# eora-ai/torchok

Measured on AMD Instinct MI355X. Metric: images/sec (node) ResNet-50 224px bs256/GPU; step p50 ms, higher is better.
Workload: dtype bf16

## Files before the change

### torchok_amd/csrc/conv_wgrad.hip

```cpp
#include "tok_common.h"
#include "conv_common.h"
#include <type_traits>
#include <stdlib.h>

namespace {

struct WgradArgs {
  const bf16* x;
  const bf16* dy;
  float* ws;
  int H, W, C, K, R, S, P, Q, stride, pad;
  int M, PQ, HW, Ktot;
  int tilesN, tilesK, splitM, mchunk;
  uint32_t x_bytes, dy_bytes;
  uint32_t pq_mul, pq_shift, q_mul, q_shift;
  float* cs;
  int cs_cols;
  int adv_q, adv_p;
  size_t cs_stride, ws_stride;
};

__device__ __forceinline__ uint32_t magic_div(uint32_t n, uint32_t mul, uint32_t shift) {
  return (uint32_t)(((uint64_t)__umulhi(n, mul) + n) >> shift);
}
// ... 663 lines not shown
  for (int st = 0; st < steps; ++st) {
    asm volatile("s_waitcnt vmcnt(%0) lgkmcnt(0)" ::"n"(LOADS) : "memory");
    __builtin_amdgcn_s_barrier();
    issue(nxt);
    const uint32_t Yb = lds_base + cur * STAGE + rbase;
    const uint32_t Xb = Yb + TILE;
    u32x2 ya[NT][2], xb[KTL][2];
#pragma unroll
    for (int i = 0; i < NT; ++i) {
      ya[i][0] = tr_read_asm(Yb + colb(i));
      ya[i][1] = tr_read_asm(Yb + 16 * 128 + colb(i));
    }
#pragma unroll
    for (int j = 0; j < KTL; ++j) {
      const int J = wv * KTL + j;
      const uint32_t ad = Xb + (uint32_t)((J >> 2) * TILE) + colb(J & 3);
      xb[j][0] = tr_read_asm(ad);
      xb[j][1] = tr_read_asm(ad + 16 * 128);
    }
    bf16x8 af[NT];
    asm volatile("s_waitcnt lgkmcnt(%0)" ::"n"(2 * (KTL - 5)) : "memory");
    __builtin_amdgcn_sched_barrier(0);
#pragma unroll
    for (int i = 0; i < NT; ++i) af[i] = __builtin_bit_cast(bf16x8, (u32x4){ya[i][0][0], ya[i][0][1], ya[i][1][0], ya[i][1][1]});
#pragma unroll
    for (int j = 0; j < 5; ++j) {
      const bf16x8 bfr = __builtin_bit_cast(bf16x8, (u32x4){xb[j][0][0], xb[j][0][1], xb[j][1][0], xb[j][1][1]});
#pragma unroll
      for (int i = 0; i < NT; ++i) acc[i][j] = __builtin_amdgcn_mfma_f32_16x16x32_bf16(af[i], bfr, acc[i][j], 0, 0, 0);
    }
    __builtin_amdgcn_sched_barrier(0);
    asm volatile("s_waitcnt lgkmcnt(0)" ::: "memory");
    __builtin_amdgcn_sched_barrier(0);
#pragma unroll
    for (int j = 5; j < KTL; ++j) {
      const bf16x8 bfr = __builtin_bit_cast(bf16x8, (u32x4){xb[j][0][0], xb[j][0][1], xb[j][1][0], xb[j][1][1]});
#pragma unroll
      for (int i = 0; i < NT; ++i) acc[i][j] = __builtin_amdgcn_mfma_f32_16x16x32_bf16(af[i], bfr, acc[i][j], 0, 0, 0);
    }
    cur = cur == NST - 1 ? 0 : cur + 1;
    nxt = nxt == NST - 1 ? 0 : nxt + 1;
  }
  asm volatile("s_waitcnt vmcnt(0)" ::: "memory");

  float* out = a.ws + (size_t)split * a.K * a.Ktot;
#pragma unroll
  for (int j = 0; j < KTL; ++j) {
    const int J = wv * KTL + j;
    const int cin = ct * TC + (J & 3) * 16 + li;
    const int kcol = (J >> 2) * a.C + cin;
#pragma unroll
    for (int i = 0; i < NT; ++i)
#pragma unroll
      for (int r = 0; r < 4; ++r) {
        const int n = tn * TN + i * 16 + g * 4 + r;
        if (n < a.K && cin < a.C) out[(size_t)n * a.Ktot + kcol] = acc[i][j][r];
      }
  }
}


template <int CT, int NST, int KTLP>
__global__ __launch_bounds__(256, 2) void conv_wgrad_winp_kernel(WgradArgs a) {
  constexpr int MS = 32, TN = 16 * CT, TC = 16 * CT, TAPS = 9;
  constexpr int WIN = MS + 2;
  constexpr int YT = MS * 128;
  constexpr int XT = 128 * 128;
  constexpr int STAGE = YT + XT;
  constexpr int LOADS = 1 + 4;
  constexpr int NT = CT, KTL = KTLP;
  constexpr int NTILES = TAPS * CT;
  constexpr int NCW = (NTILES + KTL - 1) / KTL;
  static_assert(NCW == 4 && KTL >= 7 && NST >= 3, "four compute waves");

  extern __shared__ __attribute__((aligned(16))) char smem[];

  const int tid = threadIdx.x;
  const int lane = tid & 63;
  const int wv = __builtin_amdgcn_readfirstlane(tid >> 6);

  const int tilesC = a.tilesK;
  const int ntile = a.tilesN * tilesC;
  const int id = tok_xcd_remap(blockIdx.x, ntile * a.splitM);
  const int split = id / ntile;
  const int t = id - split * ntile;
  const int tn = t / tilesC;
  const int ct = t - tn * tilesC;

  const int mstart = split * a.mchunk;
  const int mend = min(a.M, mstart + a.mchunk);
  const int steps = (mend - mstart + MS - 1) / MS;

  auto run = [&](auto WVC) {
  const int row = tid >> 3, cc = tid & 7;
  const int clog = cc ^ ((row & 3) << 1);
  const int yn = tn * TN + clog * 8;
  const bool yn_ok = yn < a.K && clog * 8 < TN;
  const int cx = ct * TC + clog * 8;
  const bool cx_ok = cx < a.C && clog * 8 < TC;
  uint32_t doff[LOADS];
  const uint32_t dinc_y = (uint32_t)(MS * a.K) * 2u;
  const uint32_t dinc_x = (uint32_t)(MS * a.C) * 2u;
  doff[0] = yn_ok ? (uint32_t)((mstart + row) * a.K + yn) * 2u : 0xC0000000u;
#pragma unroll
  for (int j = 0; j < 4; ++j) {
    const int R = row + 32 * j;
    const int win = R / WIN;
    const bool live = cx_ok && R < 3 * WIN;
    const int pix = mstart + (win - 1) * a.W - 1 + (R - win * WIN);
    doff[1 + j] = live ? (uint32_t)(pix * a.C + cx) * 2u : 0xC0000000u;
  }

  const __amdgpu_buffer_rsrc_t ysrd = __builtin_amdgcn_make_buffer_rsrc((void*)a.dy, 0, a.dy_bytes, 0x00020000);
  const __amdgpu_buffer_rsrc_t xsrd = __builtin_amdgcn_make_buffer_rsrc((void*)a.x, 0, a.x_bytes, 0x00020000);
  typedef __attribute__((address_space(3))) void lds_void;

  auto issue_piece = [&](int slot, int pc) {
    char* base = smem + slot * STAGE + wv * 1024;
    if (pc == 0) __builtin_amdgcn_raw_ptr_buffer_load_lds(ysrd, (lds_void*)base, 16, doff[0], 0, 0, 0);
    else __builtin_amdgcn_raw_ptr_buffer_load_lds(xsrd, (lds_void*)(base + YT + (pc - 1) * 4096), 16, doff[pc], 0, 0, 0);
    doff[pc] += pc == 0 ? dinc_y : dinc_x;
  };

  const int rrow = 4 * (lane >> 4) + ((lane & 15) >> 2);
  const uint32_t cq = (uint32_t)((lane & 3) * 8);
  typedef __attribute__((address_space(3))) char lds_char;
  const uint32_t lds_base = (uint32_t)(size_t)(lds_char*)smem;
  const uint32_t yrc = (uint32_t)(rrow * 128) | cq | (uint32_t)(((rrow & 3) << 1) << 4);

  int pp[2], qq[2], mm0 = mstart + rrow;
#pragma unroll
  for (int h = 0; h < 2; ++h) {
    const uint32_t mc = (uint32_t)min(mm0 + 16 * h, a.M - 1);
    const uint32_t b = magic_div(mc, a.pq_mul, a.pq_shift);
    const uint32_t rem = mc - b * (uint32_t)a.PQ;
    const uint32_t p0 = magic_div(rem, a.q_mul, a.q_shift);
    pp[h] = (int)p0; qq[h] = (int)(rem - p0 * (uint32_t)a.Q);
  }
  const int mend16 = mend - 16;

  constexpr int W0 = decltype(WVC)::value;
  constexpr int T0 = (W0 * KTL) / CT;
  auto tap_of = [](int j) constexpr { return (W0 * KTL + j) / CT - T0; };
  auto last_j = [&](int k) constexpr { int l = -1; for (int j = 0; j < KTL && W0 * KTL + j < NTILES; ++j) if (tap_of(j) == k) l = j; return l; };
  uint32_t xrc[3];
#pragma unroll
  for (int k = 0; k < 3; ++k) {
    const int tap = T0 + k < TAPS ? T0 + k : TAPS - 1;
    const int kr = tap / 3, ks = tap - kr * 3;
    const int R = kr * WIN + ks + rrow;
    xrc[k] = (uint32_t)(R * 128) | cq | (uint32_t)(((R & 3) << 1) << 4);
  }
  f32x4 acc[NT][KTL];
#pragma unroll
  for (int i = 0; i < NT; ++i)
#pragma unroll
    for (int j = 0; j < KTL; ++j) acc[i][j] = (f32x4){0.f, 0.f, 0.f, 0.f};

  auto bases_tap = [&](int slot, int k, uint32_t (&tb)[3][2]) {
    const uint32_t Xb = lds_base + slot * STAGE + YT;
    const uint32_t zero_line = Xb + 127 * 128;
    const int tap = T0 + k < TAPS ? T0 + k : TAPS - 1;
    const int kr = tap / 3, ks = tap - kr * 3;
#pragma unroll
    for (int h = 0; h < 2; ++h) {
      bool ok = h == 0 ? mm0 < mend : mm0 < mend16;
      if (kr == 0) ok = ok && pp[h] >= 1;
      if (kr == 2) ok = ok && pp[h] <= a.H - 2;
      if (ks == 0) ok = ok && qq[h] >= 1;
      if (ks == 2) ok = ok && qq[h] <= a.W - 2;
      tb[k][h] = ok ? xrc[k] + (Xb + (uint32_t)(h * 16 * 128)) : zero_line;
    }
  };
  auto advance = [&]() {
#pragma unroll
    for (int h = 0; h < 2; ++h) {
      int q = qq[h] + a.adv_q;
      const bool wq = q >= a.Q;
      q -= wq ? a.Q : 0;
      int p = pp[h] + a.adv_p + (wq ? 1 : 0);
      p -= p >= a.P ? a.P : 0;
      qq[h] = q; pp[h] = p;
    }
    mm0 += MS;
  };
  auto read_y = [&](int slot, int i, u32x2 (&ya)[NT][2]) {
    const uint32_t ad = (yrc + (lds_base + slot * STAGE)) ^ (uint32_t)(i * 32);
    asm volatile("ds_read_b64_tr_b16 %0, %1" : "=v"(ya[i][0]) : "v"(ad));
    asm volatile("ds_read_b64_tr_b16 %0, %1 offset:2048" : "=v"(ya[i][1]) : "v"(ad));
  };
  auto read_x = [&](const uint32_t (&tb)[3][2], int j, u32x2 (&xb)[KTL][2]) {
    if (W0 * KTL + j >= NTILES) return;
    const int J = W0 * KTL + j;
    const int k = J / CT - T0;
    const uint32_t tl = (uint32_t)((J % CT) * 32);
    xb[j][0] = tr_read_asm(tb[k][0] ^ tl);
    xb[j][1] = tr_read_asm(tb[k][1] ^ tl);
  };

  u32x2 yA[NT][2], yB[NT][2], xb[KTL][2];
  uint32_t tb[3][2];

#pragma unroll
  for (int s_ = 0; s_ < NST; ++s_)
#pragma unroll
    for (int pc = 0; pc < LOADS; ++pc) issue_piece(s_, pc);
  asm volatile("s_waitcnt vmcnt(%0)" ::"n"((NST - 1) * LOADS) : "memory");
  __builtin_amdgcn_s_barrier();
#pragma unroll
  for (int k = 0; k < 3; ++k) bases_tap(0, k, tb);
#pragma unroll
  for (int i = 0; i < NT; ++i) read_y(0, i, yA);
#pragma unroll
  for (int j = 0; j < KTL; ++j) read_x(tb, j, xb);
  advance();
#pragma unroll
  for (int k = 0; k < 3; ++k) bases_tap(1 % NST, k, tb);
  int rd = 1 % NST, wr = 0;

  auto body = [&](u32x2 (&ycur)[NT][2], u32x2 (&ynxt)[NT][2]) {
    asm volatile("s_waitcnt vmcnt(%0) lgkmcnt(0)" ::"n"((NST - 2) * LOADS) : "memory");
    __builtin_amdgcn_s_barrier();
    __builtin_amdgcn_sched_barrier(0);
    const int rd2 = rd == NST - 1 ? 0 : rd + 1;
    bf16x8 af[NT];
#pragma unroll
    for (int i = 0; i < NT; ++i) af[i] = __builtin_bit_cast(bf16x8, (u32x4){ycur[i][0][0], ycur[i][0][1], ycur[i][1][0], ycur[i][1][1]});
#pragma unroll
    for (int j = 0; j < KTL; ++j) {
      if (W0 * KTL + j < NTILES) {
        const bf16x8 bfr = __builtin_bit_cast(bf16x8, (u32x4){xb[j][0][0], xb[j][0][1], xb[j][1][0], xb[j][1][1]});
#pragma unroll
        for (int i = 0; i < NT; ++i) acc[i][j] = __builtin_amdgcn_mfma_f32_16x16x32_bf16(af[i], bfr, acc[i][j], 0, 0, 0);
      }
      if (j < LOADS) issue_piece(wr, j);
      if (j == 0) advance();
      if (j >= 1 && (j - 1) * 2 < NT) { read_y(rd, (j - 1) * 2, ynxt); if ((j - 1) * 2 + 1 < NT) read_y(rd, (j - 1) * 2 + 1, ynxt); }
      read_x(tb, j, xb);
#pragma unroll
      for (int k = 0; k < 3; ++k)
        if (last_j(k) == j) bases_tap(rd2, k, tb);
      __builtin_amdgcn_sched_barrier(0);
    }
    rd = rd2;
    wr = wr == NST - 1 ? 0 : wr + 1;
  };
  for (int st = 0; st < steps; st += 2) {
    body(yA, yB);
    if (st + 1 < steps) body(yB, yA);
  }
  asm volatile("s_waitcnt vmcnt(0) lgkmcnt(0)" ::: "memory");

  int lane2;
  asm volatile("v_mbcnt_lo_u32_b32 %0, -1, 0\n\tv_mbcnt_hi_u32_b32 %0, -1, %0" : "=v"(lane2));
  const int g = lane2 >> 4, li = lane2 & 15;
  float* out = a.ws + (size_t)split * a.K * a.Ktot;
#pragma unroll
  for (int j = 0; j < KTL; ++j) {
    const int J = W0 * KTL + j;
    if (J >= NTILES) continue;
    const int cin = ct * TC + (J % CT) * 16 + li;
    const int kcol = (J / CT) * a.C + cin;
#pragma unroll
    for (int i = 0; i < NT; ++i)
#pragma unroll
      for (int r = 0; r < 4; ++r) {
        const int n = tn * TN + i * 16 + g * 4 + r;
        if (n < a.K && cin < a.C) out[(size_t)n * a.Ktot + kcol] = acc[i][j][r];
      }
  }
  };
  if (wv == 0) run(std::integral_constant<int, 0>{});
  else if (wv == 1) run(std::integral_constant<int, 1>{});
  else if (wv == 2) run(std::integral_constant<int, 2>{});
  else run(std::integral_constant<int, 3>{});
}

__global__ void wgrad_reduce_kernel(const float* __restrict__ ws, float* __restrict__ dw, int splitM,
                                    int k_real, int R, int S, int c_real, int K, int S_pad,
                                    int C_pad, int accumulate) {
  const size_t total = (size_t)k_real * R * S * c_real;
  const size_t slab = (size_t)K * R * S_pad * C_pad;
  for (size_t i = (size_t)blockIdx.x * blockDim.x + threadIdx.x; i < total;
       i += (size_t)gridDim.x * blockDim.x) {
    const int c = (int)(i % c_real);
    size_t rest = i / c_real;
    const int s = (int)(rest % S);
    rest /= S;
    const int r = (int)(rest % R);
    const int k = (int)(rest / R);
    const size_t src = (((size_t)k * R + r) * S_pad + s) * C_pad + c;
    float t = 0.f;
    for (int sp = 0; sp < splitM; sp += 8) {
      float v[8];
#pragma unroll
      for (int u = 0; u < 8; ++u) v[u] = ws[(size_t)(sp + u < splitM ? sp + u : splitM - 1) * slab + src];
#pragma unroll
      for (int u = 0; u < 8; ++u) t += sp + u < splitM ? v[u] : 0.f;
    }
    dw[i] = accumulate ? dw[i] + t : t;
  }
}

template <int U>
__device__ __forceinline__ void reduce_slabs(const float* __restrict__ ws, size_t stride, size_t i, int row, int splitM, float4& t) {
  for (int sp = row; sp < splitM; sp += 16 * U) {
    float4 v[U];
#pragma unroll
    for (int u = 0; u < U; ++u) {
      const int su = sp + 16 * u;
      v[u] = reinterpret_cast<const float4*>(ws + (size_t)(su < splitM ? su : splitM - 1) * stride)[i];
    }
#pragma unroll
    for (int u = 0; u < U; ++u) {
      if (sp + 16 * u < splitM) { t.x += v[u].x; t.y += v[u].y; t.z += v[u].z; t.w += v[u].w; }
    }
  }
}

__global__ __launch_bounds__(256) void wgrad_reduce_flat_kernel(const float* __restrict__ ws, float* __restrict__ dw,
                                                                int splitM, size_t slab, int accumulate, size_t stride,
                                                                float* __restrict__ extra, int extra_n, int extra_pad,
                                                                int extra_acc) {
  __shared__ float4 red[16][16];
  const int col = threadIdx.x & 15, row = threadIdx.x >> 4;
  const size_t m4 = slab >> 2;
  const size_t n4 = m4 + (extra != nullptr ? (size_t)(extra_pad >> 2) : 0);
  for (size_t base = (size_t)blockIdx.x * 16; base < n4; base += (size_t)gridDim.x * 16) {
    const size_t i = base + col;
    float4 t = {0.f, 0.f, 0.f, 0.f};
    if (i < n4) {
      if (splitM > 64) reduce_slabs<8>(ws, stride, i, row, splitM, t);
      else if (splitM > 32) reduce_slabs<4>(ws, stride, i, row, splitM, t);
      else if (splitM > 16) reduce_slabs<2>(ws, stride, i, row, splitM, t);
      else if (row < splitM) {
        const float4 v = reinterpret_cast<const float4*>(ws + (size_t)row * stride)[i];
        t.x += v.x; t.y += v.y; t.z += v.z; t.w += v.w;
      }
    }
    red[row][col] = t;
    __syncthreads();
    for (int s_ = 8; s_ > 0; s_ >>= 1) {
      if (row < s_) {
        const float4 o = red[row + s_][col];
        float4 m = red[row][col];
        m.x += o.x; m.y += o.y; m.z += o.z; m.w += o.w;
        red[row][col] = m;
      }
      __syncthreads();
    }
    if (row == 0 && i < m4) {
      float4 r = red[0][col];
      if (accumulate) {
        const float4 o = reinterpret_cast<const float4*>(dw)[i];
        r.x += o.x; r.y += o.y; r.z += o.z; r.w += o.w;
      }
      reinterpret_cast<float4*>(dw)[i] = r;
    } else if (row == 0 && i < n4) {
      const float4 r = red[0][col];
      const float rv[4] = {r.x, r.y, r.z, r.w};
      const int e0 = (int)(i - m4) * 4;
#pragma unroll
      for (int e = 0; e < 4; ++e)
        if (e0 + e < extra_n) extra[e0 + e] = extra_acc ? extra[e0 + e] + rv[e] : rv[e];
    }
    __syncthreads();
  }
}

struct Plan {
  int TN, TK, tilesN, tilesK, splitM, mchunk, MS;
  bool ring;
  bool taps;
};

static int taps_target() {
  static const int v = [] { const char* e = getenv("TOK_WGRAD_TAPS_WGS"); return (int)(e ? atoi(e) : 256); }();
  return v;
}

static int ring_target() {
  static const int v = [] { const char* e = getenv("TOK_WGRAD_WGS"); return (int)(e ? atoi(e) : 0); }();
  return v;
}

Plan make_plan(const tok_conv_desc* d) {
  Plan p;
  const int Ktot = d->r * d->s_pad * d->c;
  const long long M = (long long)d->n * d->p * d->q;
  p.taps = false;
  const bool same3 = d->r == 3 && d->s == 3 && d->s_pad == 3 && d->stride == 1 && d->pad == 1 &&
                     (unsigned long long)d->n * d->h * d->w * d->c * 2 < 0x40000000ull &&
                     (unsigned long long)d->n * d->p * d->q * d->k * 2 < 0x40000000ull;
  const bool w64 = d->c % 64 == 0 && d->k % 64 == 0;
  const bool w48 = !w64 && d->c % 48 == 0 && d->k % 48 == 0 && same3;
  if (d->c != 4 && (w64 || w48) && d->r == 3 && d->s == 3 && d->s_pad == 3) {
    p.taps = true; p.ring = false;
    p.TN = w64 ? 64 : 48; p.TK = p.TN; p.MS = 32;
    p.tilesN = tok_cdiv(d->k, p.TN);
    p.tilesK = tok_cdiv(d->c, p.TN);
    const int tiles = p.tilesN * p.tilesK;
    long long split = (taps_target() + tiles - 1) / tiles;
    const long long max_split = (M + 8 * 32 - 1) / (8 * 32);
    if (split > max_split) split = max_split;
    if (split > 512) split = 512;
    if (split < 1) split = 1;
    long long chunk = (M + split - 1) / split;
    chunk = ((chunk + 31) / 32) * 32;
    p.mchunk = (int)chunk;
    p.splitM = (int)((M + chunk - 1) / chunk);
    return p;
  }
  p.ring = d->c != 4 && d->r == 1 && d->s == 1 && d->stride == 1 && d->pad == 0;
  if (p.ring) {
    p.MS = 32;
    if (d->k <= 64) { p.TN = 64; p.TK = Ktot >= 256 ? 256 : (Ktot >= 128 ? 128 : 64); }
    else if (Ktot <= 64) { p.TK = 64; p.TN = d->k >= 256 ? 256 : 128; }
    else { p.TN = 128; p.TK = 128; }
    static const int big = [] { const char* e = getenv("TOK_WGRAD_256"); return (int)(e ? atoi(e) : 1); }();
    if (big && d->r == 1 && d->s == 1 && d->stride == 1 && d->pad == 0 && d->k >= 256 && Ktot >= 256 && M >= (big >= 2 ? 8192 : 200000) &&
        (long long)tok_cdiv(d->k, 256) * tok_cdiv(Ktot, 256) * 65536 * 2 <= (long long)d->k * Ktot * 3) {
      p.TN = 256; p.TK = 256;
    }
    p.tilesN = tok_cdiv(d->k, p.TN);
    p.tilesK = tok_cdiv(Ktot, p.TK);
    const int tiles = p.tilesN * p.tilesK;
    const int stage = 32 * (p.TN + p.TK) * 2;
    const int per_cu = (160 * 1024) / (3 * stage);
    static const int long_target = [] { const char* e = getenv("TOK_WGRAD_WGS_LONG"); return (int)(e ? atoi(e) : 0); }();
    const int target = (long_target > 0 && M >= 100000) ? long_target
                       : ring_target() > 0 ? ring_target() : 256 * (per_cu > 2 ? 2 : per_cu);
    long long split = (target + tiles - 1) / tiles;
    const long long max_split = (M + 8 * 32 - 1) / (8 * 32);
    if (split > max_split) split = max_split;
    if (split > 512) split = 512;
    if (split < 1) split = 1;
    long long chunk = (M + split - 1) / split;
    chunk = ((chunk + 31) / 32) * 32;
    p.mchunk = (int)chunk;
    p.splitM = (int)((M + chunk - 1) / chunk);
    return p;
  }
  p.TN = d->k >= 128 ? 128 : 64;
  p.TK = Ktot >= 128 ? 128 : 64;
  p.tilesN = tok_cdiv(d->k, p.TN);
  p.tilesK = tok_cdiv(Ktot, p.TK);
  const int tiles = p.tilesN * p.tilesK;
  static const int tb_target = [] { const char* e = getenv("TOK_WGRAD_2BUF_WGS"); return (int)(e ? atoi(e) : 1024); }();
  long long split = (tb_target + tiles - 1) / tiles;
  p.MS = (M >= 100000 && p.TN == 128 && p.TK == 128) ? 64 : 32;
  const long long max_split = (M + 8 * p.MS - 1) / (8 * p.MS);
  if (split > max_split) split = max_split;
  const long long cap = (d->c == 4 && tiles <= 2) ? 512 : 256;
  if (split > cap) split = cap;
  if (split < 1) split = 1;
  long long chunk = (M + split - 1) / split;
  chunk = ((chunk + p.MS - 1) / p.MS) * p.MS;
  p.mchunk = (int)chunk;
  p.splitM = (int)((M + chunk - 1) / chunk);
  return p;
}

template <int TN, int TK>
void launch_ring(const WgradArgs& a, hipStream_t st) {
  constexpr int smem = 3 * 32 * (TN + TK) * 2;
  static const bool attr_set = [&] {
    (void)hipFuncSetAttribute(reinterpret_cast<const void*>(&conv_wgrad_ring_kernel<TN, TK>),
                              hipFuncAttributeMaxDynamicSharedMemorySize, smem);
    return true;
  }();
  (void)attr_set;
  hipLaunchKernelGGL((conv_wgrad_ring_kernel<TN, TK>), dim3(a.tilesN * a.tilesK * a.splitM), dim3(256), smem, st, a);
}

template <int TN, int TK, bool C4, int MS, bool PWK>
void launch_wgrad_pw(const WgradArgs& a, hipStream_t st) {
  constexpr int smem = 2 * MS * ((TN + 16) * 2 + (TK + 16) * 2);
  static const bool attr_set = [&] {
    (void)hipFuncSetAttribute(reinterpret_cast<const void*>(&conv_wgrad_kernel<TN, TK, C4, MS, PWK>),
                              hipFuncAttributeMaxDynamicSharedMemorySize, smem);
    return true;
  }();
  (void)attr_set;
  hipLaunchKernelGGL((conv_wgrad_kernel<TN, TK, C4, MS, PWK>), dim3(a.tilesN * a.tilesK * a.splitM), dim3(256),
                     smem, st, a);
}

template <int TN, int TK, bool C4, int MS>
void launch_wgrad_ms(const WgradArgs& a, hipStream_t st) {
  if constexpr (!C4) {
    if (a.R == 1 && a.S == 1 && a.stride == 1 && a.pad == 0) { launch_wgrad_pw<TN, TK, C4, MS, true>(a, st); return; }
  }
  launch_wgrad_pw<TN, TK, C4, MS, false>(a, st);
}

template <int TN, int TK, bool C4>
void launch_wgrad(const WgradArgs& a, hipStream_t st, int ms) {
  if (ms == 64) launch_wgrad_ms<TN, TK, C4, 64>(a, st);
  else launch_wgrad_ms<TN, TK, C4, 32>(a, st);
}

}

extern "C" size_t tok_conv_wgrad_ws_bytes(const tok_conv_desc* d) {
  if (d == nullptr) return 0;
  const Plan p = make_plan(d);
  return (size_t)p.splitM * d->k * d->r * d->s_pad * d->c * sizeof(float);
}

extern "C" int tok_conv_wgrad_bias_ok(const tok_conv_desc* d) {
  if (d == nullptr || d->c == 4) return 0;
  return make_plan(d).ring ? 1 : 0;
}

extern "C" size_t tok_conv_wgrad_bias_ws_bytes(const tok_conv_desc* d) {
  if (d == nullptr) return 0;
  const Plan p = make_plan(d);
  return tok_conv_wgrad_ws_bytes(d) + (size_t)p.splitM * d->k * sizeof(float);
}

namespace {
int wgrad_impl(const tok_conv_desc* d, const void* x, const void* dy, float* dw, int k_real, int c_real, void* ws, size_t ws_bytes,
               int accumulate, float* dbias, int bias_accumulate, void* stream);
}

extern "C" int tok_conv_wgrad(const tok_conv_desc* d, const void* x, const void* dy, float* dw,
                              int k_real, int c_real, void* ws, size_t ws_bytes, int accumulate,
                              void* stream) {
  return wgrad_impl(d, x, dy, dw, k_real, c_real, ws, ws_bytes, accumulate, nullptr, 0, stream);
}

extern "C" int tok_conv_wgrad_bias(const tok_conv_desc* d, const void* x, const void* dy, float* dw, int k_real, int c_real,
                                   void* ws, size_t ws_bytes, int accumulate, float* dbias, int bias_accumulate, void* stream) {
  TOK_CHECK_ARG(dbias != nullptr, "tok_conv_wgrad_bias: dbias must not be null");
  TOK_CHECK_ARG(tok_conv_wgrad_bias_ok(d), "tok_conv_wgrad_bias: layer not served (ask tok_conv_wgrad_bias_ok)");
  return wgrad_impl(d, x, dy, dw, k_real, c_real, ws, ws_bytes, accumulate, dbias, bias_accumulate, stream);
}

namespace {
int wgrad_impl(const tok_conv_desc* d, const void* x, const void* dy, float* dw, int k_real, int c_real, void* ws, size_t ws_bytes,
               int accumulate, float* dbias, int bias_accumulate, void* stream) {
  TOK_CHECK_ARG(d && x && dy && dw && ws, "tok_conv_wgrad: null pointer");
  if (tok_dbg_skip(16)) return TOK_OK;
  TOK_CHECK_ARG(d->k % 8 == 0 && (d->c % 8 == 0 || d->c == 4), "tok_conv_wgrad: bad channel padding");
  TOK_CHECK_ARG(k_real <= d->k && c_real <= d->c, "tok_conv_wgrad: real dims exceed padded dims");
  TOK_CHECK_ARG(d->c == 4 ? d->s_pad == 8 : d->s_pad == d->s, "tok_conv_wgrad: bad s_pad");
  const Plan p = make_plan(d);
  const size_t need = dbias ? tok_conv_wgrad_bias_ws_bytes(d) : tok_conv_wgrad_ws_bytes(d);
  if (ws_bytes < need) {
    tok_set_error("tok_conv_wgrad: workspace %zu < %zu bytes", ws_bytes, need);
    return TOK_ERR_WORKSPACE;
  }
  const bool flat = (k_real == d->k) && (c_real == d->c) && (d->s_pad == d->s) &&
                    (((size_t)d->k * d->r * d->s * d->c) % 4 == 0) && (((uintptr_t)dw & 15) == 0);
  const bool direct = flat && p.splitM == 1 && !accumulate;
  WgradArgs a;
  a.x = (const bf16*)x; a.dy = (const bf16*)dy; a.ws = direct ? dw : (float*)ws;
  a.H = d->h; a.W = d->w; a.C = d->c; a.K = d->k; a.R = d->r; a.S = d->s_pad; a.P = d->p; a.Q = d->q;
  a.stride = d->stride; a.pad = d->pad;
  a.M = d->n * d->p * d->q; a.PQ = d->p * d->q; a.HW = d->h * d->w;
  make_magic((uint32_t)a.PQ, a.pq_mul, a.pq_shift);
  make_magic((uint32_t)d->q, a.q_mul, a.q_shift);
  a.adv_q = 32 % d->q; a.adv_p = (32 / d->q) % d->p;
  a.Ktot = d->r * d->s_pad * d->c;
  a.tilesN = p.tilesN; a.tilesK = p.tilesK; a.splitM = p.splitM; a.mchunk = p.mchunk;
  const size_t slab_f = (size_t)d->k * d->r * d->s_pad * d->c;
  const int cs_pad = (k_real + 3) / 4 * 4;
  const bool cs_inline = dbias != nullptr && flat && !direct;
  a.ws_stride = cs_inline ? slab_f + cs_pad : slab_f;
  a.cs = dbias ? (cs_inline ? (float*)ws + slab_f : (float*)((char*)ws + tok_conv_wgrad_ws_bytes(d))) : nullptr;
  a.cs_stride = cs_inline ? a.ws_stride : (size_t)k_real;
  a.cs_cols = k_real;
  {
    const unsigned long long xb = (unsigned long long)d->n * d->h * d->w * d->c * 2;
    const unsigned long long yb = (unsigned long long)a.M * d->k * 2;
    TOK_CHECK_ARG(xb < 0xFFFFFFF0ull && yb < 0xFFFFFFF0ull, "tok_conv_wgrad: tensors of 4 GiB or more are not supported");
    a.x_bytes = (uint32_t)xb; a.dy_bytes = (uint32_t)yb;
  }
  hipStream_t st = tok_stream(stream);
  const bool c4 = d->c == 4;
  if (c4 && dbias == nullptr && stem_wgrad_serves(d)) {
    stem_wgrad_launch(d, x, dy, a.ws, p.splitM, st);
  } else
  if (p.taps) {
    constexpr int smem = 3 * 10 * 32 * 128;
    static const bool attr_set = [&] {
      (void)hipFuncSetAttribute(reinterpret_cast<const void*>(&conv_wgrad_taps_kernel<0>),
                                hipFuncAttributeMaxDynamicSharedMemorySize, smem);
      return true;
    }();
    (void)attr_set;
    const bool same = a.stride == 1 && a.pad == 1 && a.P == a.H && a.Q == a.W && a.x_bytes < 0x40000000u && a.dy_bytes < 0x40000000u;
    if (same) {
      constexpr int smem_p = 3 * (32 * 128 + 128 * 128);
      static const bool attr_p = [&] {
        (void)hipFuncSetAttribute(reinterpret_cast<const void*>(&conv_wgrad_winp_kernel<4, 3, 9>), hipFuncAttributeMaxDynamicSharedMemorySize, smem_p);
        (void)hipFuncSetAttribute(reinterpret_cast<const void*>(&conv_wgrad_winp_kernel<3, 3, 7>), hipFuncAttributeMaxDynamicSharedMemorySize, smem_p);
        return true;
      }();
      (void)attr_p;
      const dim3 gw(a.tilesN * a.tilesK * a.splitM);
      if (p.TN == 48) hipLaunchKernelGGL((conv_wgrad_winp_kernel<3, 3, 7>), gw, dim3(256), smem_p, st, a);
      else hipLaunchKernelGGL((conv_wgrad_winp_kernel<4, 3, 9>), gw, dim3(256), smem_p, st, a);
    } else {
      hipLaunchKernelGGL((conv_wgrad_taps_kernel<0>), dim3(a.tilesN * a.tilesK * a.splitM), dim3(256), smem, st, a);
    }
  } else if (p.ring) {
    if (p.TN == 256 && p.TK == 256) {
      constexpr int smem8 = 3 * 32 * (256 + 256) * 2;
      static const bool attr8 = [] {
        (void)hipFuncSetAttribute(reinterpret_cast<const void*>(&conv_wgrad_ring8_kernel<256, 256>),
                                  hipFuncAttributeMaxDynamicSharedMemorySize, smem8);
        return true;
      }();
      (void)attr8;
      hipLaunchKernelGGL((conv_wgrad_ring8_kernel<256, 256>), dim3(a.tilesN * a.tilesK * a.splitM), dim3(512), smem8, st, a);
    }
    else if (p.TN == 64 && p.TK == 64) launch_ring<64, 64>(a, st);
    else if (p.TN == 64 && p.TK == 128) launch_ring<64, 128>(a, st);
    else if (p.TN == 64 && p.TK == 256) launch_ring<64, 256>(a, st);
    else if (p.TN == 128 && p.TK == 64) launch_ring<128, 64>(a, st);
    else if (p.TN == 256 && p.TK == 64) launch_ring<256, 64>(a, st);
    else launch_ring<128, 128>(a, st);
  } else if (p.TN == 128 && p.TK == 128) {
    if (c4) launch_wgrad<128, 128, true>(a, st, p.MS); else launch_wgrad<128, 128, false>(a, st, p.MS);
  } else if (p.TN == 128) {
    if (c4) launch_wgrad<128, 64, true>(a, st, p.MS); else launch_wgrad<128, 64, false>(a, st, p.MS);
  } else if (p.TK == 128) {
    if (c4) launch_wgrad<64, 128, true>(a, st, p.MS); else launch_wgrad<64, 128, false>(a, st, p.MS);
  } else {
    if (c4) launch_wgrad<64, 64, true>(a, st, p.MS); else launch_wgrad<64, 64, false>(a, st, p.MS);
  }
  TOK_CHECK_LAUNCH("tok_conv_wgrad");
  if (dbias != nullptr && !cs_inline) {
    if (int e = tok_colsum_f32(a.cs, p.splitM, k_real, dbias, bias_accumulate, stream)) return e;
  }
  if (direct) return TOK_OK;
  if (flat) {
    if (tok_dbg_skip(2)) return TOK_OK;
    const size_t slab = (size_t)d->k * d->r * d->s * d->c;
    const size_t nb = (slab / 4 + 15) / 16;
    hipLaunchKernelGGL(wgrad_reduce_flat_kernel, dim3((int)(nb < 4096 ? nb : 4096)), dim3(256), 0, st,
                       (const float*)ws, dw, p.splitM, slab, accumulate, cs_inline ? a.ws_stride : slab,
                       cs_inline ? dbias : (float*)nullptr, k_real, cs_inline ? cs_pad : 0, bias_accumulate);
    TOK_CHECK_LAUNCH("tok_conv_wgrad(reduce)");
    return TOK_OK;
  }
  const size_t total = (size_t)k_real * d->r * d->s * c_real;
  const int blocks = (int)((total + 255) / 256 < 2048 ? (total + 255) / 256 : 2048);
  hipLaunchKernelGGL(wgrad_reduce_kernel, dim3(blocks), dim3(256), 0, st, (const float*)ws, dw,
                     p.splitM, k_real, d->r, d->s, c_real, d->k, d->s_pad, d->c, accumulate);
  TOK_CHECK_LAUNCH("tok_conv_wgrad(reduce)");
  return TOK_OK;
}
}
```

Baseline: 14600.

## Rewrite split-M wgrad reduction as per-thread register fold without shared memory

Replaces the shared-memory tree reduction of split-M workspace slabs with a kernel where each thread owns V contiguous outputs and folds all slabs itself into 16 register accumulators, followed by an in-register tree. Vector width (1/2/4) and unroll depth are chosen on the host from the output size and splitM, so small layers get more threads. This removes __syncthreads and LDS traffic and launches one thread per output vector instead of a grid-stride loop. In exchange, each thread serially reads every slab, which lowers parallelism when splitM is large and raises register pressure.

```diff
diff --git a/torchok_amd/csrc/conv_wgrad.hip b/torchok_amd/csrc/conv_wgrad.hip
--- a/torchok_amd/csrc/conv_wgrad.hip
+++ b/torchok_amd/csrc/conv_wgrad.hip
@@ -989,70 +989,84 @@
   }
 }
 
-template <int U>
-__device__ __forceinline__ void reduce_slabs(const float* __restrict__ ws, size_t stride, size_t i, int row, int splitM, float4& t) {
-  for (int sp = row; sp < splitM; sp += 16 * U) {
-    float4 v[U];
-#pragma unroll
-    for (int u = 0; u < U; ++u) {
-      const int su = sp + 16 * u;
-      v[u] = reinterpret_cast<const float4*>(ws + (size_t)(su < splitM ? su : splitM - 1) * stride)[i];
-    }
-#pragma unroll
-    for (int u = 0; u < U; ++u) {
-      if (sp + 16 * u < splitM) { t.x += v[u].x; t.y += v[u].y; t.z += v[u].z; t.w += v[u].w; }
-    }
-  }
-}
-
+template <int V> struct FoldVec;
+template <> struct FoldVec<1> { float f[1]; };
+template <> struct alignas(8) FoldVec<2> { float f[2]; };
+template <> struct alignas(16) FoldVec<4> { float f[4]; };
+
+template <int V, int B, bool TAIL>
+__device__ __forceinline__ void fold_round(const float* __restrict__ src, size_t stride, int sp, int splitM, float (&acc)[16][V]) {
+  FoldVec<V> v[B];
+#pragma unroll
+  for (int u = 0; u < B; ++u) {
+    const int s = TAIL && sp + u >= splitM ? splitM - 1 : sp + u;
+    v[u] = *reinterpret_cast<const FoldVec<V>*>(src + (size_t)s * stride);
+  }
+#pragma unroll
+  for (int u = 0; u < B; ++u) {
+    if (!TAIL || sp + u < splitM) {
+#pragma unroll
+      for (int j = 0; j < V; ++j) acc[u & 15][j] += v[u].f[j];
+    }
+  }
+}
+
+template <int V, int B>
 __global__ __launch_bounds__(256) void wgrad_reduce_flat_kernel(const float* __restrict__ ws, float* __restrict__ dw,
                                                                 int splitM, size_t slab, int accumulate, size_t stride,
                                                                 float* __restrict__ extra, int extra_n, int extra_pad,
                                                                 int extra_acc) {
-  __shared__ float4 red[16][16];
-  const int col = threadIdx.x & 15, row = threadIdx.x >> 4;
-  const size_t m4 = slab >> 2;
-  const size_t n4 = m4 + (extra != nullptr ? (size_t)(extra_pad >> 2) : 0);
-  for (size_t base = (size_t)blockIdx.x * 16; base < n4; base += (size_t)gridDim.x * 16) {
-    const size_t i = base + col;
-    float4 t = {0.f, 0.f, 0.f, 0.f};
-    if (i < n4) {
-      if (splitM > 64) reduce_slabs<8>(ws, stride, i, row, splitM, t);
-      else if (splitM > 32) reduce_slabs<4>(ws, stride, i, row, splitM, t);
-      else if (splitM > 16) reduce_slabs<2>(ws, stride, i, row, splitM, t);
-      else if (row < splitM) {
-        const float4 v = reinterpret_cast<const float4*>(ws + (size_t)row * stride)[i];
-        t.x += v.x; t.y += v.y; t.z += v.z; t.w += v.w;
-      }
-    }
-    red[row][col] = t;
-    __syncthreads();
-    for (int s_ = 8; s_ > 0; s_ >>= 1) {
-      if (row < s_) {
-        const float4 o = red[row + s_][col];
-        float4 m = red[row][col];
-        m.x += o.x; m.y += o.y; m.z += o.z; m.w += o.w;
-        red[row][col] = m;
-      }
-      __syncthreads();
-    }
-    if (row == 0 && i < m4) {
-      float4 r = red[0][col];
-      if (accumulate) {
-        const float4 o = reinterpret_cast<const float4*>(dw)[i];
-        r.x += o.x; r.y += o.y; r.z += o.z; r.w += o.w;
-      }
-      reinterpret_cast<float4*>(dw)[i] = r;
-    } else if (row == 0 && i < n4) {
-      const float4 r = red[0][col];
-      const float rv[4] = {r.x, r.y, r.z, r.w};
-      const int e0 = (int)(i - m4) * 4;
-#pragma unroll
-      for (int e = 0; e < 4; ++e)
-        if (e0 + e < extra_n) extra[e0 + e] = extra_acc ? extra[e0 + e] + rv[e] : rv[e];
-    }
-    __syncthreads();
-  }
+  static_assert(B % 16 == 0, "a round is whole passes over the 16 rows");
+  const size_t n = slab + (extra != nullptr ? (size_t)extra_pad : 0);
+  const size_t e = ((size_t)blockIdx.x * 256 + threadIdx.x) * V;
+  if (e >= n) return;
+  float acc[16][V];
+#pragma unroll
+  for (int r = 0; r < 16; ++r)
+#pragma unroll
+    for (int j = 0; j < V; ++j) acc[r][j] = 0.f;
+  const float* src = ws + e;
+  int sp = 0;
+  for (; sp + B <= splitM; sp += B) fold_round<V, B, false>(src, stride, sp, splitM, acc);
+  if (sp < splitM) fold_round<V, B, true>(src, stride, sp, splitM, acc);
+#pragma unroll
+  for (int h = 8; h > 0; h >>= 1)
+#pragma unroll
+    for (int r = 0; r < h; ++r)
+#pragma unroll
+      for (int j = 0; j < V; ++j) acc[r][j] += acc[r + h][j];
+  if (e < slab) {
+    FoldVec<V> r;
+#pragma unroll
+    for (int j = 0; j < V; ++j) r.f[j] = acc[0][j];
+    if (accumulate) {
+      const FoldVec<V> o = *reinterpret_cast<const FoldVec<V>*>(dw + e);
+#pragma unroll
+      for (int j = 0; j < V; ++j) r.f[j] += o.f[j];
+    }
+    *reinterpret_cast<FoldVec<V>*>(dw + e) = r;
+  } else {
+    const int e0 = (int)(e - slab);
+#pragma unroll
+    for (int j = 0; j < V; ++j)
+      if (e0 + j < extra_n) extra[e0 + j] = extra_acc ? extra[e0 + j] + acc[0][j] : acc[0][j];
+  }
+}
+
+void launch_reduce_flat(const float* ws, float* dw, int splitM, size_t slab, int accumulate, size_t stride, float* extra,
+                        int extra_n, int extra_pad, int extra_acc, hipStream_t st) {
+  const size_t n = slab + (extra != nullptr ? (size_t)extra_pad : 0);
+  const int V = (n >= (1u << 17) || splitM <= 16) ? 4 : (n >= (1u << 16) || splitM <= 32) ? 2 : 1;
+  const dim3 grid((unsigned)((n / V + 255) / 256));
+  if (V == 4)
+    hipLaunchKernelGGL((wgrad_reduce_flat_kernel<4, 16>), grid, dim3(256), 0, st, ws, dw, splitM, slab, accumulate, stride, extra,
+                       extra_n, extra_pad, extra_acc);
+  else if (V == 2)
+    hipLaunchKernelGGL((wgrad_reduce_flat_kernel<2, 32>), grid, dim3(256), 0, st, ws, dw, splitM, slab, accumulate, stride, extra,
+                       extra_n, extra_pad, extra_acc);
+  else
+    hipLaunchKernelGGL((wgrad_reduce_flat_kernel<1, 64>), grid, dim3(256), 0, st, ws, dw, splitM, slab, accumulate, stride, extra,
+                       extra_n, extra_pad, extra_acc);
 }
 
 struct Plan {
@@ -1326,10 +1340,8 @@
   if (flat) {
     if (tok_dbg_skip(2)) return TOK_OK;
     const size_t slab = (size_t)d->k * d->r * d->s * d->c;
-    const size_t nb = (slab / 4 + 15) / 16;
-    hipLaunchKernelGGL(wgrad_reduce_flat_kernel, dim3((int)(nb < 4096 ? nb : 4096)), dim3(256), 0, st,
-                       (const float*)ws, dw, p.splitM, slab, accumulate, cs_inline ? a.ws_stride : slab,
-                       cs_inline ? dbias : (float*)nullptr, k_real, cs_inline ? cs_pad : 0, bias_accumulate);
+    launch_reduce_flat((const float*)ws, dw, p.splitM, slab, accumulate, cs_inline ? a.ws_stride : slab,
+                       cs_inline ? dbias : (float*)nullptr, k_real, cs_inline ? cs_pad : 0, bias_accumulate, st);
     TOK_CHECK_LAUNCH("tok_conv_wgrad(reduce)");
     return TOK_OK;
   }
```

Result: no change. 14690, median of 6 (+0.6%).
